# ericyinyzy/VQAttack

Hardware: AMD Instinct MI355X
Metric: adversarial_vqa_examples_per_sec (higher is better)
Workload: dtype f32; 1 GPU; vlmo_base VQAttack image PGD (BASELINE configs[1]): batch 64 per GPU, 40 PGD steps, 384x384 images, questions of 6..14 real tokens ([CLS] + n words + [SEP], n ~ U{4..12} seeded) padded to 40 (the all-padding columns are not run through the encoder), eps 0.125 step 0.01 L-inf clip [-1,1], random start, sanity_checks on, black-box scoring + ASR gather; batch_per_gpu=64, pgd_steps=40, image_size=384, text_len=40, substitutable_words=0

## Files before the change

### include/vqattack_hip.h

```cpp
#ifndef VQATTACK_HIP_H
#define VQATTACK_HIP_H

#include <stddef.h>
#include <stdint.h>

#ifdef __cplusplus
extern "C" {
#endif

typedef void* vqa_stream_t;

#define VQA_OK 0
#define VQA_ERR_NULL (-1)
#define VQA_ERR_SHAPE (-2)
#define VQA_ERR_ALIGN (-3)

#define VQA_CLIP 1u
#define VQA_CHECK_RANGE 2u
#define VQA_FLAG_RANGE 1
#define VQA_FLAG_BAD_LABEL 2
#define VQA_FLAG_DEGENERATE 4

int vqa_abi_version(void);
const char* vqa_error_string(int code);
// ... 54 lines not shown
int vqa_neg_cos_max_layers(void);
int vqa_neg_cos_rows_multi(const float* const* a, const float* const* b, float* const* ga, int n_layers,
                           float* partial, const uint8_t* row_mask, long mask_period, long rows0, long rows1, int D,
                           long a_stride0, long a_stride1, long b_stride0, long b_stride1, long g_stride0,
                           long g_stride1, float gscale, float cos_eps, float* loss_out, int accumulate,
                           vqa_stream_t stream);

int vqa_sum_partials(const float* partial, int count, float* dst, int accumulate, float scale,
                     vqa_stream_t stream);

int vqa_ce_max_label_sets(void);
long vqa_ce_scratch_floats(int K, long groups);
int vqa_ce_rows(const float* logits, long row_stride, const int64_t* labels, int K, long rows, int V,
                long ignore_index, long rows_per_group, float* scratch, float* grad, float* row_loss, float gscale,
                float* loss_out, int accumulate, int* flag, unsigned char* row_state, vqa_stream_t stream);

int vqa_gather_rows(const float* src, const int64_t* idx, float* dst, int B, int L, int K, int D,
                    vqa_stream_t stream);

int vqa_cand_dir_sim(const float* word, const float* pos, const float* type, const float* gamma,
                     const float* beta, float ln_eps, const float* e_ori, const float* grad,
                     const int32_t* cand, float* out, int n_cand, int L, int K, int D, vqa_stream_t stream);

int vqa_embed_tokens(const float* word, const float* pos, const float* type, const float* gamma, const float* beta,
                     float ln_eps, const int32_t* triples, int n, float* dst, int D, vqa_stream_t stream);

int vqa_greedy_accept(const int32_t* cand, const int32_t* order, const int32_t* seg, int B, int L,
                      const int64_t* ori_ids, int64_t* cur_ids, int32_t* new_id, int32_t* acc_rank, const float* table,
                      int V, int E, float threshold, vqa_stream_t stream);

int vqa_attn_fwd(const float* q, const float* k, const float* v, const float* bias, float* o, float* lse, float* scores,
                 int B, int H, int Sq, int Sk, const long* strides, const long* bias_strides, float scale,
                 const int* key_hole, int nsplit, float* split_ws, vqa_stream_t stream);
long vqa_attn_scores_floats(int B, int H, int Sq, int Sk);
long vqa_attn_split_ws_floats(int B, int H, int Sq, int Sk, int nsplit);

int vqa_attn_bwd(const float* q, const float* k, const float* v, const float* bias, const float* o, const float* go,
                 const float* lse, const float* scores, float* delta, float* dq, float* dk, float* dv, float* ds_ws, int B,
                 int H, int Sq, int Sk, const long* strides, const long* bias_strides, const long* grad_strides,
                 float scale, int nsplit, float* split_ws, vqa_stream_t stream);
long vqa_attn_bwd_ws_floats(int B, int H, int Sq, int Sk);

int vqa_resize_bicubic_h_u8(const uint8_t* src, int h, int w_in, int c, const int32_t* kk, const int32_t* bounds,
                            int ksize, int w_out, uint8_t* dst, vqa_stream_t stream);
int vqa_resize_bicubic_v_normalize(const uint8_t* src, int h_in, int w, int c, const int32_t* kk,
                                   const int32_t* bounds, int ksize, int h_out, float mean, float stdv, float* dst,
                                   vqa_stream_t stream);

int vqa_ln_fwd(const float* x, const float* r0, const float* r1, const float* rscale, float* x_out,
               const float* gamma0, const float* beta0, const float* gamma1, const float* beta1, float* y0, float* y1,
               float* mean, float* rstd, long rows, int D, long period, long split, float eps, vqa_stream_t stream);
int vqa_ln_bwd(const float* dy0, const float* dy1, const float* x, const float* mean, const float* rstd,
               const float* gamma0, const float* gamma1, const float* g_a, const float* g_inj, const float* rscale,
               float* dx, float* dr0, float* dr1, long rows, int D, long period, long split, vqa_stream_t stream);
int vqa_ln_bwd_post(const float* dy_a, const float* dy_b, const float* g_inj, const float* s, const float* rstd,
                    const float* gamma, float* ds, long rows, int D, vqa_stream_t stream);
int vqa_gelu_fwd(const float* h, float* a, size_t n, vqa_stream_t stream);
int vqa_gelu_bwd(const float* h, const float* da, float* dh, size_t n, vqa_stream_t stream);

size_t vqa_gemm_packed_bytes(int K, int N);
int vqa_gemm_pack_b(const float* w, long ldw, int trans, void* packed, int K, int N, vqa_stream_t stream);
int vqa_gemm_bf16x6(const float* A, long lda, const void* packed, const float* bias, float* C, long ldc, long M, int N,
                    int K, vqa_stream_t stream);

size_t vqa_gemm_small_ws_bytes(long M, int N, int ksplit);
int vqa_gemm_bf16x6_small(const float* A, long lda, const void* packed, const float* bias, float* C, long ldc, long M,
// ... 7 lines not shown
```

### vqattack_amd/_hip.py

```python
import ctypes
import os
import threading

import torch

_HERE = os.path.dirname(os.path.abspath(__file__))
LIB_PATH = os.path.join(_HERE, "lib", "libvqattack_hip.so")
TUNING_LIB_PATH = os.path.join(_HERE, "lib", "libvqattack_hip_tuning.so")

VQA_CLIP = 1
VQA_CHECK_RANGE = 2
VQA_FLAG_RANGE = 1
VQA_FLAG_BAD_LABEL = 2
VQA_FLAG_DEGENERATE = 4
ABI_VERSION = 4

_c_float_p = ctypes.c_void_p
_sz = ctypes.c_size_t
_f = ctypes.c_float
_i = ctypes.c_int
_u = ctypes.c_uint
_l = ctypes.c_long
_p = ctypes.c_void_p

SIGNATURES = {
    "vqa_abi_version": (_i, []),
    "vqa_error_string": (ctypes.c_char_p, [_i]),
    "vqa_linf_init": (_i, [_p, _p, _p, _sz, _f, _f, _f, _u, _p, _p]),
    "vqa_linf_fgm": (_i, [_p, _p, _p, _sz, _f, _f, _f, _u, _p, _p]),
    "vqa_linf_step": (_i, [_p, _p, _p, _p, _sz, _f, _f, _f, _f, _u, _p, _p]),
    "vqa_linf_project": (_i, [_p, _p, _p, _sz, _f, _f, _f, _u, _p]),
    "vqa_clip_eta_linf": (_i, [_p, _p, _sz, _f, _p]),
    "vqa_optimize_linear_linf": (_i, [_p, _p, _sz, _f, _p]),
    "vqa_zero_out_clipped_grads": (_i, [_p, _p, _p, _sz, _f, _f, _p]),
    "vqa_reduce_ws_bytes": (_sz, [_i, _sz]),
    "vqa_sumsq_per_sample": (_i, [_p, _p, _p, _i, _sz, _p, _p]),
    "vqa_absmax_ties_per_sample": (_i, [_p, _p, _p, _i, _sz, _p, _p]),
    "vqa_l2_fgm": (_i, [_p, _p, _p, _p, _i, _sz, _f, _f, _f, _u, _p, _p]),
    "vqa_l2_project": (_i, [_p, _p, _p, _p, _i, _sz, _f, _f, _f, _u, _p]),
    "vqa_l1_fgm": (_i, [_p, _p, _p, _p, _p, _i, _sz, _f, _f, _f, _u, _p, _p]),
    "vqa_scale_per_sample": (_i, [_p, _p, _p, _p, _i, _sz, _f, _i, _p, _p]),
    "vqa_neg_cos_partials": (_i, []),
    "vqa_neg_cos_rows": (_i, [_p, _p, _p, _p, _p, _l, _l, _l, _i, _l, _l, _l, _l, _l, _l, _f, _f, _p, _i, _p]),
    "vqa_neg_cos_max_layers": (_i, []),
    "vqa_neg_cos_rows_multi": (_i, [_p, _p, _p, _i, _p, _p, _l, _l, _l, _i, _l, _l, _l, _l, _l, _l, _f, _f, _p, _i, _p]),
    "vqa_sum_partials": (_i, [_p, _i, _p, _i, _f, _p]),
    "vqa_ce_max_label_sets": (_i, []),
    "vqa_ce_scratch_floats": (_l, [_i, _l]),
    "vqa_ce_rows": (_i, [_p, _l, _p, _i, _l, _i, _l, _l, _p, _p, _p, _f, _p, _i, _p, _p, _p]),
    "vqa_gather_rows": (_i, [_p, _p, _p, _i, _i, _i, _i, _p]),
    "vqa_cand_dir_sim": (_i, [_p, _p, _p, _p, _p, _f, _p, _p, _p, _p, _i, _i, _i, _i, _p]),
    "vqa_embed_tokens": (_i, [_p, _p, _p, _p, _p, _f, _p, _i, _p, _i, _p]),
    "vqa_greedy_accept": (_i, [_p, _p, _p, _i, _i, _p, _p, _p, _p, _p, _i, _i, _f, _p]),
    "vqa_attn_fwd": (_i, [_p, _p, _p, _p, _p, _p, _p, _i, _i, _i, _i, _p, _p, _f, _p, _i, _p, _p]),
    "vqa_attn_split_ws_floats": (_l, [_i, _i, _i, _i, _i]),
    "vqa_attn_scores_floats": (_l, [_i, _i, _i, _i]),
    "vqa_attn_bwd": (_i, [_p, _p, _p, _p, _p, _p, _p, _p, _p, _p, _p, _p, _p, _i, _i, _i, _i, _p, _p, _p, _f, _i, _p, _p]),
    "vqa_attn_bwd_ws_floats": (_l, [_i, _i, _i, _i]),
    "vqa_ln_fwd": (_i, [_p] * 13 + [_l, _i, _l, _l, _f, _p]),
    "vqa_ln_bwd": (_i, [_p] * 13 + [_l, _i, _l, _l, _p]),
    "vqa_ln_bwd_post": (_i, [_p] * 7 + [_l, _i, _p]),
    "vqa_gelu_fwd": (_i, [_p, _p, _sz, _p]),
    "vqa_gelu_bwd": (_i, [_p, _p, _p, _sz, _p]),
    "vqa_resize_bicubic_h_u8": (_i, [_p, _i, _i, _i, _p, _p, _i, _i, _p, _p]),
    "vqa_resize_bicubic_v_normalize": (_i, [_p, _i, _i, _i, _p, _p, _i, _i, _f, _f, _p, _p]),
    "vqa_gemm_packed_bytes": (_sz, [_i, _i]),
    "vqa_gemm_pack_b": (_i, [_p, _l, _i, _p, _i, _i, _p]),
    "vqa_gemm_bf16x6": (_i, [_p, _l, _p, _p, _p, _l, _l, _i, _i, _p]),
    "vqa_gemm_small_ws_bytes": (_sz, [_l, _i, _i]),
    "vqa_gemm_bf16x6_small": (_i, [_p, _l, _p, _p, _p, _l, _l, _i, _i, _i, _p, _p]),
}

_lib = None
_lock = threading.Lock()


class HipExtensionError(RuntimeError):
    pass


def load_library(path=None):
    tuning = os.environ.get("VQA_TUNING_LIB", "") not in ("", "0")
    if path is None:
        path = TUNING_LIB_PATH if tuning else LIB_PATH
    if not os.path.exists(path):
        raise HipExtensionError(
            "HIP kernel library not found at {} -- build it with `python -m vqattack_amd.build` "
# ... 79 lines not shown
```

### vqattack_amd/attention.py

```python
import ctypes

import torch

from . import _hip
from ._hip import check, lib, ptr, stream_for

HEAD_DIM = 64


def _bshd(t, name):
    if not t.is_cuda or t.dtype != torch.float32 or t.dim() != 4 or t.shape[-1] != HEAD_DIM:
        raise _hip.HipExtensionError("{} must be a float32 (B, S, H, 64) HIP tensor, got {} {}".format(
            name, t.dtype, tuple(t.shape)))
    if t.stride(-1) != 1 or any(s % 4 for s in t.stride()[:-1]) or t.data_ptr() % 16:
        t = t.contiguous()
    return t


def _bias_view(bias, b, h, sq, sk):
    if bias is None:
        return None, None
    if bias.dtype != torch.float32 or not bias.is_cuda:
        raise TypeError("bias must be a float32 HIP tensor")
    bias, in_place = _bias_layout(bias, sk)
# ... 34 lines not shown

    def dense(self):
        sk = self.slab.shape[-1]
        b = self.hole.shape[0]
        keys = torch.arange(sk, device=self.slab.device)
        masked = (keys[None, :] >= self.hole[:, :1]) & (keys[None, :] < self.hole[:, 1:2])
        pad = torch.zeros(b, 1, 1, sk, device=self.slab.device).masked_fill(masked[:, None, None, :], float("-inf"))
        return self.slab + pad


def _split_hole(bias):
    if isinstance(bias, KeyHoleBias):
        return bias.slab, bias.hole
    return bias, None


_CUS = {}


def loop_split(b, h, sq, sk, device, backward=True):
    import os
    pinned = os.environ.get("VQA_ATTN_SPLIT")
    tiles = ((min(sq, sk) if backward else sk) + 31) // 32
    if pinned:
        return max(1, min(int(pinned), tiles))
    dev = torch.device(device).index or 0
    if dev not in _CUS:
        _CUS[dev] = torch.cuda.get_device_properties(dev).multi_processor_count
    wgs = b * h * ((max(sq, sk) + 127) // 128)
    want = 2 * _CUS[dev]
    if wgs * 2 > want:
        return 1
    return max(1, min(8, tiles // 2, -(-want // wgs)))


def _split_ws(b, h, sq, sk, nsplit, device):
    if nsplit <= 1:
        return None
    return torch.empty(int(lib().vqa_attn_split_ws_floats(b, h, sq, sk, nsplit)), dtype=torch.float32, device=device)


def _forward(q, k, v, bias, bstr, scale, save_scores=False, key_hole=None):
    b, sq, h, _ = q.shape
    sk = k.shape[1]
    nsplit = loop_split(b, h, sq, sk, q.device, backward=False)
    sws = _split_ws(b, h, sq, sk, nsplit, q.device)
    o = torch.empty((b, sq, h, HEAD_DIM), dtype=torch.float32, device=q.device)
    lse = torch.empty((b, h, sq), dtype=torch.float32, device=q.device)
    scores = None
    if save_scores:
        if scores_fit(b, h, sq, sk):
            scores = torch.empty(int(lib().vqa_attn_scores_floats(b, h, sq, sk)), dtype=torch.float32, device=q.device)
        elif key_hole is not None:
            raise _hip.HipExtensionError("a key hole needs the saved-scores backward (the recomputing forms read the "
                                         "padding from the bias): pass KeyHoleBias.dense() at this size")
    strides = _longs([q.stride(0), q.stride(1), q.stride(2), k.stride(0), k.stride(1), k.stride(2),
                      v.stride(0), v.stride(1), v.stride(2), o.stride(0), o.stride(1), o.stride(2)])
    if key_hole is not None and (key_hole.dtype != torch.int32 or tuple(key_hole.shape) != (b, 2) or
                                 not key_hole.is_cuda or not key_hole.is_contiguous()):
        raise TypeError("key_hole must be a contiguous int32 (B, 2) HIP tensor")
    with torch.cuda.device(q.device):
        check(lib().vqa_attn_fwd(ptr(q), ptr(k), ptr(v), ptr(bias), ptr(o), ptr(lse), ptr(scores), b, h, sq, sk, strides,
                                 _longs(bstr) if bstr else None, scale,
                                 None if key_hole is None else ctypes.c_void_p(key_hole.data_ptr()), nsplit, ptr(sws),
                                 stream_for(q)),
              "vqa_attn_fwd")
    return o, lse, scores


def scores_fit(b, h, sq, sk):
    n = int(lib().vqa_attn_scores_floats(b, h, sq, sk))
    return 0 < 4 * n <= SCORES_LIMIT and 0 < 4 * int(lib().vqa_attn_bwd_ws_floats(b, h, sq, sk)) <= DS_WORKSPACE_LIMIT


def _prepare(q, k, v, bias, scale, need_grad=False):
    q, k, v = _bshd(q, "q"), _bshd(k, "k"), _bshd(v, "v")
    b, sq, h, _ = q.shape
    sk = k.shape[1]
    if k.shape != (b, sk, h, HEAD_DIM) or v.shape != k.shape:
        raise ValueError("q / k / v shape mismatch: {} {} {}".format(tuple(q.shape), tuple(k.shape), tuple(v.shape)))
    hole = None
    if isinstance(bias, KeyHoleBias):
        if need_grad and not scores_fit(b, h, sq, sk):
            bias = bias.dense()
        else:
            bias, hole = bias.slab, bias.hole
    bias, bstr = _bias_view(bias, b, h, sq, sk)
    return q, k, v, bias, bstr, HEAD_DIM ** -0.5 if scale is None else float(scale), hole


def attention_forward(q, k, v, bias=None, scale=None):
    q, k, v, bias, bstr, scale, hole = _prepare(q, k, v, bias, scale)
    return _forward(q, k, v, bias, bstr, scale, key_hole=hole)[:2]


DS_WORKSPACE_LIMIT = 8 << 30
SCORES_LIMIT = 6 << 30


# ... 80 lines not shown
```

### vqattack_amd/build.py

```python
import os
import shutil
import subprocess
import sys

HERE = os.path.dirname(os.path.abspath(__file__))
SRC_DIR = os.path.join(HERE, "csrc")
LIB_DIR = os.path.join(HERE, "lib")
LIB_PATH = os.path.join(LIB_DIR, "libvqattack_hip.so")
TUNING_LIB_PATH = os.path.join(LIB_DIR, "libvqattack_hip_tuning.so")
SOURCES = ["linf.hip", "lnorm.hip", "loss.hip", "ce.hip", "text.hip", "image.hip", "attn.hip", "block.hip", "gemm.hip"]
FLAGS = ["-O3", "--offload-arch=gfx950", "-ffp-contract=off", "-fPIC", "-shared", "-std=c++17",
         "-Wall", "-Wno-unused-function"]


KERNEL_SOURCES = (("stream4_kernel", "linf.hip"), ("neg_cos_rows", "loss.hip"), ("ce_rows", "ce.hip"), ("ce_count", "ce.hip"),
                  ("attn_", "attn.hip"), ("sumsq", "lnorm.hip"), ("absmax", "lnorm.hip"), ("per_sample", "lnorm.hip"),
                  ("sum_stage2", "lnorm.hip"), ("ln_fwd", "block.hip"), ("ln_bwd", "block.hip"), ("gelu", "block.hip"),
                  ("resize", "image.hip"), ("gather_rows", "text.hip"), ("cand_dir_sim", "text.hip"),
                  ("embed_tokens", "text.hip"), ("greedy_accept", "text.hip"), ("gemm_", "gemm.hip"))


def kernel_source_digest(kernel_name):
    import hashlib
    src = next((f for key, f in KERNEL_SOURCES if key in kernel_name), None)
    if src is None:
        return None
    h = hashlib.sha256(" ".join(FLAGS).encode())
    for path in (os.path.join(SRC_DIR, src), os.path.join(SRC_DIR, "common.hpp"),
                 os.path.join(HERE, "..", "include", "vqattack_hip.h")):
        with open(path, "rb") as fh:
            h.update(fh.read())
    return h.hexdigest()


def _hipcc():
    for cand in (os.environ.get("HIPCC"), shutil.which("hipcc"), "/opt/rocm/bin/hipcc"):
        if cand and os.path.exists(cand):
            return cand
    raise RuntimeError("hipcc not found: the HIP kernels of vqattack_amd cannot be built")


def _stale(path=LIB_PATH):
    if not os.path.exists(path):
        return True
    built = os.path.getmtime(path)
    deps = [os.path.join(SRC_DIR, f) for f in os.listdir(SRC_DIR)]
    deps.append(os.path.join(HERE, "..", "include", "vqattack_hip.h"))
    return any(os.path.getmtime(d) > built for d in deps)


def build(force=False, verbose=False, tuning=False):
    target = TUNING_LIB_PATH if tuning else LIB_PATH
    if not force and not _stale(target):
        return target
    os.makedirs(LIB_DIR, exist_ok=True)
    cmd = [_hipcc()] + FLAGS + (["-DVQA_TUNING"] if tuning else []) + \
        [os.path.join(SRC_DIR, s) for s in SOURCES] + ["-o", target + ".tmp"]
    if verbose:
        print(" ".join(cmd))
    proc = subprocess.run(cmd, capture_output=True, text=True)
    if proc.returncode != 0:
# ... 13 lines not shown
```

### vqattack_amd/csrc/attn.hip

```cpp
#include "common.hpp"

namespace vqa {

typedef float f32x4 __attribute__((ext_vector_type(4)));
typedef float f32x16 __attribute__((ext_vector_type(16)));

constexpr int kTile = 32;
constexpr int kKs = 65;

struct AttnDims {
  int B, H, Sq, Sk;
  long q_sb, q_ss, q_sh;
  long k_sb, k_ss, k_sh;
  long v_sb, v_ss, v_sh;
  long o_sb, o_ss, o_sh;
  long bias_sb, bias_sh, bias_sr;
  float scale;
};

#ifdef VQA_TUNING
__device__ int d_attn_ablate = 0;
#define VQA_ABLATE(bit) (d_attn_ablate & (bit))
__device__ unsigned long long* d_attn_stamps = nullptr;
#define VQA_STAMP_DECL unsigned long long stamp_t = 0, stamp_sum[8] = {0, 0, 0, 0, 0, 0, 0, 0}; const bool stamp_on = d_attn_stamps != nullptr;
#define VQA_STAMP_START()                                                                              \
  do {                                                                                                 \
    if (stamp_on) {                                                                                    \
      __builtin_amdgcn_sched_barrier(0);                                                               \
      asm volatile("s_memtime %0\n\ts_waitcnt lgkmcnt(0)" : "=s"(stamp_t)::"memory");                  \
      __builtin_amdgcn_sched_barrier(0);                                                               \
    }                                                                                                  \
  } while (0)
#define VQA_STAMP(seg)                                                                                 \
// ... 261 lines not shown
        const float m_new = grow ? mx : m;
        const float mc_new = m_new * kLog2e;
        const float alpha = m == -INFINITY ? 0.0f : __builtin_amdgcn_exp2f(mc - mc_new);
        m = m_new;
        mc = grow ? mc_new : mc;
        l *= alpha;
#pragma unroll
        for (int i = 0; i < 16; ++i) {
          o0[i] *= alpha;
          o1[i] *= alpha;
        }
      }
#pragma unroll
      for (int i = 0; i < 16; ++i) {
        st[i] = __builtin_amdgcn_exp2f(__builtin_fmaf(st[i], kLog2e, -mc));
        l += st[i];
      }
      VQA_STAMP(2);
#pragma unroll
      for (int i = 0; i < 16; ++i) {
        const f32x2 vv = *reinterpret_cast<const f32x2*>(Vs + ((i & 3) + 8 * (i >> 2)) * kVi);
        o0 = mfma(vv[0], st[i], o0);
        o1 = mfma(vv[1], st[i], o1);
      }
      VQA_STAMP(3);
      bcur = bnext;
    }
    if (more) {
      store_tile<kKs>(Kbuf[(kt + 1) & 1], tk, 1.0f);
      store_tile_interleaved(Vbuf[(kt + 1) & 1], tv, 1.0f);
    }
    VQA_STAMP(4);
    if (STORE_S && active && !VQA_ABLATE(1)) {
#pragma unroll
      for (int g = 0; g < 4; ++g)
        *reinterpret_cast<f32x4*>(scp + static_cast<long>(kt) * kBlockFloats + 256 * g) =
            f32x4{sraw[4 * g], sraw[4 * g + 1], sraw[4 * g + 2], sraw[4 * g + 3]};
    }
    VQA_STAMP(5);
    __syncthreads();
    VQA_STAMP(6);
  }
  if (active) VQA_STAMP_FLUSH(0, n_tiles - t_lo);
  if (SPLIT) {
    if (qi < d.Sq) {
      l = halves_sum(l);
      const long row = (static_cast<long>(b) * d.H + head) * d.Sq + qi;
      float* wo = sp.ws + (row * nsp + part) * 64;
#pragma unroll
      for (int g = 0; g < 4; ++g) {
        const int dim = 8 * g + 4 * h;
        *reinterpret_cast<f32x4*>(wo + dim) = f32x4{o0[4 * g], o0[4 * g + 1], o0[4 * g + 2], o0[4 * g + 3]};
        *reinterpret_cast<f32x4*>(wo + 32 + dim) = f32x4{o1[4 * g], o1[4 * g + 1], o1[4 * g + 2], o1[4 * g + 3]};
      }
      if (h == 0) {
        float* ml = sp.ws + static_cast<long>(d.B) * d.H * d.Sq * nsp * 64 + (row * nsp + part) * 2;
        ml[0] = m == -INFINITY ? -INFINITY : mc;
        ml[1] = l;
      }
    }
    return;
  }
  if (qi < d.Sq) {
    l = halves_sum(l);
    const float inv = 1.0f / l;
    float* op = o + b * d.o_sb + head * d.o_sh + static_cast<long>(qi) * d.o_ss;
// ... 511 lines not shown
static int check_attn(const float* q, const float* k, const float* v, const AttnDims& d) {
  if (!q || !k || !v) return VQA_ERR_NULL;
  if (d.B < 0 || d.H <= 0 || d.Sq <= 0 || d.Sk <= 0 || d.H > 65535 || d.B > 65535) return VQA_ERR_SHAPE;
  const long blocks = ((d.Sq > d.Sk ? d.Sq : d.Sk) + 127L) / 128;
  if (blocks * d.H * d.B > 2147483647L) return VQA_ERR_SHAPE;
  if ((d.q_sb | d.q_ss | d.q_sh | d.k_sb | d.k_ss | d.k_sh | d.v_sb | d.v_ss | d.v_sh | d.o_sb | d.o_ss | d.o_sh) & 3)
    return VQA_ERR_SHAPE;
  if (!aligned16(q) || !aligned16(k) || !aligned16(v)) return VQA_ERR_ALIGN;
  return VQA_OK;
}

long vqa_attn_scores_floats(int B, int H, int Sq, int Sk) {
  if (B < 0 || H <= 0 || Sq <= 0 || Sk <= 0) return 0;
  return static_cast<long>(B) * H * sc_rows(Sq) * sc_pitch(Sk);
}

long vqa_attn_split_ws_floats(int B, int H, int Sq, int Sk, int nsplit) {
  if (B < 0 || H <= 0 || Sq <= 0 || Sk <= 0 || nsplit < 1) return 0;
  if (nsplit == 1) return 0;
  const long rq = static_cast<long>(B) * H * Sq, rk = static_cast<long>(B) * H * Sk;
  const long fwd = split_fwd_floats(rq, nsplit), dkv = 2 * split_sum_floats(rk, nsplit), dq = split_sum_floats(rq, nsplit);
  return fwd > dkv ? (fwd > dq ? fwd : dq) : (dkv > dq ? dkv : dq);
}

static int check_split(int nsplit, const float* split_ws, int tiles, long wgs) {
  if (nsplit < 1) return VQA_ERR_SHAPE;
  if (nsplit == 1) return VQA_OK;
  if (!split_ws) return VQA_ERR_NULL;
  if (!aligned16(split_ws)) return VQA_ERR_ALIGN;
  if (nsplit > tiles || wgs * nsplit > 2147483647L) return VQA_ERR_SHAPE;
  return VQA_OK;
}

int vqa_attn_fwd(const float* q, const float* k, const float* v, const float* bias, float* o, float* lse, float* scores,
                 int B, int H, int Sq, int Sk, const long* strides, const long* bias_strides, float scale,
                 const int* key_hole, int nsplit, float* split_ws, vqa_stream_t stream) {
  clear_stale_error();
  if (!strides || !o || !lse || (bias && !bias_strides)) return VQA_ERR_NULL;
  AttnDims d{B, H, Sq, Sk, strides[0], strides[1], strides[2], strides[3], strides[4], strides[5], strides[6],
             strides[7], strides[8], strides[9], strides[10], strides[11], 0, 0, 0, scale};
  if (bias) {
    d.bias_sb = bias_strides[0];
    d.bias_sh = bias_strides[1];
    d.bias_sr = bias_strides[2];
    if (((d.bias_sb | d.bias_sh | d.bias_sr) & 3) || !aligned16(bias)) return VQA_ERR_ALIGN;
  }
  int rc = check_attn(q, k, v, d);
  if (rc != VQA_OK) return rc;
  if (!aligned16(o) || !aligned16(scores)) return VQA_ERR_ALIGN;
  const long wgs = ((Sq + 127L) / 128) * H * B;
  rc = check_split(nsplit, split_ws, (Sk + kTile - 1) / kTile, wgs);
  if (rc != VQA_OK) return rc;
  if (B == 0) return VQA_OK;
  const dim3 grid(static_cast<unsigned>(wgs * nsplit));
  hipStream_t st = static_cast<hipStream_t>(stream);
  const SplitArgs sp{nsplit, split_ws};
  if (nsplit > 1) {
    if (bias && scores) attn_fwd_kernel<true, true, true><<<grid, kBlock, 0, st>>>(q, k, v, bias, o, lse, scores, d, key_hole, sp);
    else if (bias) attn_fwd_kernel<true, false, true><<<grid, kBlock, 0, st>>>(q, k, v, bias, o, lse, scores, d, key_hole, sp);
    else if (scores) attn_fwd_kernel<false, true, true><<<grid, kBlock, 0, st>>>(q, k, v, bias, o, lse, scores, d, key_hole, sp);
    else attn_fwd_kernel<false, false, true><<<grid, kBlock, 0, st>>>(q, k, v, bias, o, lse, scores, d, key_hole, sp);
    const long rows = static_cast<long>(B) * H * Sq;
    attn_fwd_combine_kernel<<<dim3(static_cast<unsigned>((rows + kBlock / 16 - 1) / (kBlock / 16))), kBlock, 0, st>>>(
        split_ws, nsplit, o, lse, d);
    return launch_status();
  }
  if (bias && scores) attn_fwd_kernel<true, true><<<grid, kBlock, 0, st>>>(q, k, v, bias, o, lse, scores, d, key_hole, sp);
  else if (bias) attn_fwd_kernel<true, false><<<grid, kBlock, 0, st>>>(q, k, v, bias, o, lse, scores, d, key_hole, sp);
  else if (scores) attn_fwd_kernel<false, true><<<grid, kBlock, 0, st>>>(q, k, v, bias, o, lse, scores, d, key_hole, sp);
  else attn_fwd_kernel<false, false><<<grid, kBlock, 0, st>>>(q, k, v, bias, o, lse, scores, d, key_hole, sp);
  return launch_status();
}

long vqa_attn_bwd_ws_floats(int B, int H, int Sq, int Sk) {
  if (B < 0 || H <= 0 || Sq <= 0 || Sk <= 0) return 0;
  return static_cast<long>(B) * H * ds_rows(Sk) * ds_pitch(Sq);
}

int vqa_attn_bwd(const float* q, const float* k, const float* v, const float* bias, const float* o, const float* go,
                 const float* lse, const float* scores, float* delta, float* dq, float* dk, float* dv, float* ds_ws, int B,
                 int H, int Sq, int Sk, const long* strides, const long* bias_strides, const long* grad_strides,
                 float scale, int nsplit, float* split_ws, vqa_stream_t stream) {
  clear_stale_error();
  if (!strides || !grad_strides || !o || !go || !lse || !delta || !dq || !dk || !dv || (bias && !bias_strides))
    return VQA_ERR_NULL;
  AttnDims d{B, H, Sq, Sk, strides[0], strides[1], strides[2], strides[3], strides[4], strides[5], strides[6],
             strides[7], strides[8], strides[9], strides[10], strides[11], 0, 0, 0, scale};
  if (bias) {
    d.bias_sb = bias_strides[0];
    d.bias_sh = bias_strides[1];
    d.bias_sr = bias_strides[2];
    if (((d.bias_sb | d.bias_sh | d.bias_sr) & 3) || !aligned16(bias)) return VQA_ERR_ALIGN;
    if (d.bias_sr < 0 || (static_cast<long>(Sq) + 4) * d.bias_sr + Sk >= 2147483647L) return VQA_ERR_SHAPE;
  }
  const int rc = check_attn(q, k, v, d);
  if (rc != VQA_OK) return rc;
  long any = 0;
  for (int i = 0; i < 12; ++i) any |= grad_strides[i];
  if (any & 3) return VQA_ERR_SHAPE;
  if (!aligned16(o) || !aligned16(go) || !aligned16(dq) || !aligned16(dk) || !aligned16(dv) || !aligned16(ds_ws) ||
      !aligned16(scores))
    return VQA_ERR_ALIGN;
  if (ds_ws && (ds_rows(Sk) * ds_pitch(Sq) >= 2147483647L || sc_rows(Sq) * sc_pitch(Sk) >= 2147483647L))
    return VQA_ERR_SHAPE;
// ... 73 lines not shown
```

### vqattack_amd/csrc/gemm.hip

```cpp
#include "common.hpp"

namespace vqa {

typedef __bf16 bf16x8 __attribute__((ext_vector_type(8)));
typedef __bf16 bf16x2 __attribute__((ext_vector_type(2)));
typedef float f32x4 __attribute__((ext_vector_type(4)));
typedef float f32x2 __attribute__((ext_vector_type(2)));

constexpr int kGemmBM = 256, kGemmBN = 128, kGemmBK = 32;
constexpr int kGemmThreads = 512;
constexpr int kGemmMT = kGemmBM / 16, kGemmNT = kGemmBN / 16;
constexpr int kTileBytes = 64 * 16;
constexpr int kGemmABytes = kGemmMT * 3 * kTileBytes;
constexpr int kGemmBBytes = kGemmNT * 3 * kTileBytes;
constexpr int kGemmStage = kGemmABytes + kGemmBBytes;
constexpr int kGemmBPieces = kGemmBBytes / 16 / kGemmThreads;

__device__ __forceinline__ void split2(f32x2 a, bf16x2& h0, bf16x2& h1, bf16x2& h2) {
  h0 = __builtin_convertvector(a, bf16x2);
  f32x2 r = a - __builtin_convertvector(h0, f32x2);
  r.x = __builtin_isfinite(r.x) ? r.x : 0.0f;
  r.y = __builtin_isfinite(r.y) ? r.y : 0.0f;
  h1 = __builtin_convertvector(r, bf16x2);
  h2 = __builtin_convertvector(r - __builtin_convertvector(h1, f32x2), bf16x2);
}

__device__ __forceinline__ void split8(const f32x4& lo, const f32x4& hi, bf16x8& p0, bf16x8& p1, bf16x8& p2) {
  bf16x2 a[4], b[4], c[4];
  split2(f32x2{lo.x, lo.y}, a[0], b[0], c[0]);
  split2(f32x2{lo.z, lo.w}, a[1], b[1], c[1]);
  split2(f32x2{hi.x, hi.y}, a[2], b[2], c[2]);
  split2(f32x2{hi.z, hi.w}, a[3], b[3], c[3]);
  p0 = bf16x8{a[0].x, a[0].y, a[1].x, a[1].y, a[2].x, a[2].y, a[3].x, a[3].y};
  p1 = bf16x8{b[0].x, b[0].y, b[1].x, b[1].y, b[2].x, b[2].y, b[3].x, b[3].y};
  p2 = bf16x8{c[0].x, c[0].y, c[1].x, c[1].y, c[2].x, c[2].y, c[3].x, c[3].y};
}

struct GemmArgs {
  const float* A;
  const bf16x8* B;
  const float* bias;
  float* C;
  long lda, ldc, M;
  int N, K;
};

__global__ __launch_bounds__(kGemmThreads) void gemm_bf16x6_kernel(GemmArgs g) {
  __shared__ __attribute__((aligned(16))) char smem[2 * kGemmStage];
  const int tid = threadIdx.x, lane = tid & 63, wave = tid >> 6;
  const int wm = wave >> 1, wn = wave & 1;
  const int ntb = g.N / kGemmBN;
  const int mtb = static_cast<int>((g.M + kGemmBM - 1) / kGemmBM);
  const int nwg = mtb * ntb, orig = blockIdx.x, xcd = orig & 7, q = nwg >> 3, rem = nwg & 7;
  const int wg = (xcd < rem ? xcd * (q + 1) : rem * (q + 1) + (xcd - rem) * q) + (orig >> 3);
  const int mb = wg / ntb, nb = wg - mb * ntb;
  const long m0 = static_cast<long>(mb) * kGemmBM;
  const int n0 = nb * kGemmBN;
  const int nk = g.K / kGemmBK;
  const int nt16 = g.N / 16;

  const float* arow[2];
#pragma unroll
  for (int j = 0; j < 2; ++j) {
    long r = m0 + (2 * wave + j) * 16 + (lane & 15);
    r = r < g.M ? r : g.M - 1;
    arow[j] = g.A + r * g.lda + 8 * (lane >> 4);
  }
  const bf16x8* bsrc = g.B + static_cast<size_t>(nb) * kGemmNT * 3 * 64;
  const size_t bstep = static_cast<size_t>(nt16) * 3 * 64;
// ... 291 lines not shown
```

Before: 14.31 examples/s.

## Add bf16x6 split-precision MFMA attention forward kernel as default for long queries

Adds a forward attention kernel that splits fp32 Q, K, V and the probabilities into three bf16 pieces and accumulates six bf16 MFMA products per tile. K and V tiles are split into LDS once per tile, double-buffered, with the next tile prefetched into registers. The kernel is selected by default when nsplit is 1 and Sq is at least 128, except when the backward pass recomputes scores. The aim is to replace slower fp32 arithmetic with bf16 matrix-core throughput while keeping near-fp32 accuracy, at the cost of extra split work and LDS traffic. Split helpers move to a shared header.

After: 14.44 examples/s, median of 6. About the same (+1.0%).

```diff
diff --git a/include/vqattack_hip.h b/include/vqattack_hip.h
--- a/include/vqattack_hip.h
+++ b/include/vqattack_hip.h
@@ -110,6 +110,9 @@
 int vqa_attn_fwd(const float* q, const float* k, const float* v, const float* bias, float* o, float* lse, float* scores,
                  int B, int H, int Sq, int Sk, const long* strides, const long* bias_strides, float scale,
                  const int* key_hole, int nsplit, float* split_ws, vqa_stream_t stream);
+int vqa_attn_fwd_bf16x6(const float* q, const float* k, const float* v, const float* bias, float* o, float* lse,
+                        float* scores, int B, int H, int Sq, int Sk, const long* strides, const long* bias_strides,
+                        float scale, const int* key_hole, int nsplit, float* split_ws, vqa_stream_t stream);
 long vqa_attn_scores_floats(int B, int H, int Sq, int Sk);
 long vqa_attn_split_ws_floats(int B, int H, int Sq, int Sk, int nsplit);
 
diff --git a/vqattack_amd/_hip.py b/vqattack_amd/_hip.py
--- a/vqattack_amd/_hip.py
+++ b/vqattack_amd/_hip.py
@@ -53,6 +53,7 @@
     "vqa_embed_tokens": (_i, [_p, _p, _p, _p, _p, _f, _p, _i, _p, _i, _p]),
     "vqa_greedy_accept": (_i, [_p, _p, _p, _i, _i, _p, _p, _p, _p, _p, _i, _i, _f, _p]),
     "vqa_attn_fwd": (_i, [_p, _p, _p, _p, _p, _p, _p, _i, _i, _i, _i, _p, _p, _f, _p, _i, _p, _p]),
+    "vqa_attn_fwd_bf16x6": (_i, [_p, _p, _p, _p, _p, _p, _p, _i, _i, _i, _i, _p, _p, _f, _p, _i, _p, _p]),
     "vqa_attn_split_ws_floats": (_l, [_i, _i, _i, _i, _i]),
     "vqa_attn_scores_floats": (_l, [_i, _i, _i, _i]),
     "vqa_attn_bwd": (_i, [_p, _p, _p, _p, _p, _p, _p, _p, _p, _p, _p, _p, _p, _i, _i, _i, _i, _p, _p, _p, _f, _i, _p, _p]),
diff --git a/vqattack_amd/attention.py b/vqattack_amd/attention.py
--- a/vqattack_amd/attention.py
+++ b/vqattack_amd/attention.py
@@ -90,6 +90,19 @@
     if wgs * 2 > want:
         return 1
     return max(1, min(8, tiles // 2, -(-want // wgs)))
+
+
+FWD_BF16X6_DEFAULT = lambda nsplit, sq: nsplit == 1 and sq >= 128
+
+
+def _forward_entry(nsplit, sq, recomputing_backward):
+    import os
+    mode = os.environ.get("VQA_ATTN", "")
+    if mode not in ("", "fp32", "bf16x6"):
+        raise ValueError("VQA_ATTN must be 'fp32' or 'bf16x6', got '{}'".format(mode))
+    if not recomputing_backward and (mode == "bf16x6" or (mode == "" and FWD_BF16X6_DEFAULT(nsplit, sq))):
+        return lib().vqa_attn_fwd_bf16x6, "vqa_attn_fwd_bf16x6"
+    return lib().vqa_attn_fwd, "vqa_attn_fwd"
 
 
 def _split_ws(b, h, sq, sk, nsplit, device):
@@ -117,12 +130,13 @@
     if key_hole is not None and (key_hole.dtype != torch.int32 or tuple(key_hole.shape) != (b, 2) or
                                  not key_hole.is_cuda or not key_hole.is_contiguous()):
         raise TypeError("key_hole must be a contiguous int32 (B, 2) HIP tensor")
+    entry, name = _forward_entry(nsplit, sq, save_scores and scores is None)
     with torch.cuda.device(q.device):
-        check(lib().vqa_attn_fwd(ptr(q), ptr(k), ptr(v), ptr(bias), ptr(o), ptr(lse), ptr(scores), b, h, sq, sk, strides,
-                                 _longs(bstr) if bstr else None, scale,
-                                 None if key_hole is None else ctypes.c_void_p(key_hole.data_ptr()), nsplit, ptr(sws),
-                                 stream_for(q)),
-              "vqa_attn_fwd")
+        check(entry(ptr(q), ptr(k), ptr(v), ptr(bias), ptr(o), ptr(lse), ptr(scores), b, h, sq, sk, strides,
+                    _longs(bstr) if bstr else None, scale,
+                    None if key_hole is None else ctypes.c_void_p(key_hole.data_ptr()), nsplit, ptr(sws),
+                    stream_for(q)),
+              name)
     return o, lse, scores
 
 
diff --git a/vqattack_amd/build.py b/vqattack_amd/build.py
--- a/vqattack_amd/build.py
+++ b/vqattack_amd/build.py
@@ -26,7 +26,7 @@
     if src is None:
         return None
     h = hashlib.sha256(" ".join(FLAGS).encode())
-    for path in (os.path.join(SRC_DIR, src), os.path.join(SRC_DIR, "common.hpp"),
+    for path in (os.path.join(SRC_DIR, src), os.path.join(SRC_DIR, "common.hpp"), os.path.join(SRC_DIR, "split.hpp"),
                  os.path.join(HERE, "..", "include", "vqattack_hip.h")):
         with open(path, "rb") as fh:
             h.update(fh.read())
diff --git a/vqattack_amd/csrc/attn.hip b/vqattack_amd/csrc/attn.hip
--- a/vqattack_amd/csrc/attn.hip
+++ b/vqattack_amd/csrc/attn.hip
@@ -1,4 +1,7 @@
+#include <type_traits>
+
 #include "common.hpp"
+#include "split.hpp"
 
 namespace vqa {
 
@@ -326,6 +329,244 @@
     }
     VQA_STAMP(4);
     if (STORE_S && active && !VQA_ABLATE(1)) {
+#pragma unroll
+      for (int g = 0; g < 4; ++g)
+        *reinterpret_cast<f32x4*>(scp + static_cast<long>(kt) * kBlockFloats + 256 * g) =
+            f32x4{sraw[4 * g], sraw[4 * g + 1], sraw[4 * g + 2], sraw[4 * g + 3]};
+    }
+    VQA_STAMP(5);
+    __syncthreads();
+    VQA_STAMP(6);
+  }
+  if (active) VQA_STAMP_FLUSH(0, n_tiles - t_lo);
+  if (SPLIT) {
+    if (qi < d.Sq) {
+      l = halves_sum(l);
+      const long row = (static_cast<long>(b) * d.H + head) * d.Sq + qi;
+      float* wo = sp.ws + (row * nsp + part) * 64;
+#pragma unroll
+      for (int g = 0; g < 4; ++g) {
+        const int dim = 8 * g + 4 * h;
+        *reinterpret_cast<f32x4*>(wo + dim) = f32x4{o0[4 * g], o0[4 * g + 1], o0[4 * g + 2], o0[4 * g + 3]};
+        *reinterpret_cast<f32x4*>(wo + 32 + dim) = f32x4{o1[4 * g], o1[4 * g + 1], o1[4 * g + 2], o1[4 * g + 3]};
+      }
+      if (h == 0) {
+        float* ml = sp.ws + static_cast<long>(d.B) * d.H * d.Sq * nsp * 64 + (row * nsp + part) * 2;
+        ml[0] = m == -INFINITY ? -INFINITY : mc;
+        ml[1] = l;
+      }
+    }
+    return;
+  }
+  if (qi < d.Sq) {
+    l = halves_sum(l);
+    const float inv = 1.0f / l;
+    float* op = o + b * d.o_sb + head * d.o_sh + static_cast<long>(qi) * d.o_ss;
+#pragma unroll
+    for (int g = 0; g < 4; ++g) {
+      const int dim = 8 * g + 4 * h;
+      f32x4 a = {o0[4 * g] * inv, o0[4 * g + 1] * inv, o0[4 * g + 2] * inv, o0[4 * g + 3] * inv};
+      f32x4 c = {o1[4 * g] * inv, o1[4 * g + 1] * inv, o1[4 * g + 2] * inv, o1[4 * g + 3] * inv};
+      *reinterpret_cast<f32x4*>(op + dim) = a;
+      *reinterpret_cast<f32x4*>(op + 32 + dim) = c;
+    }
+    if (h == 0) lse[(static_cast<long>(b) * d.H + head) * d.Sq + qi] = mc * kLn2 + __logf(l);
+  }
+}
+
+
+constexpr int kXkPlane = 4 * kWave;
+constexpr int kXvPlane = 2 * 2 * kWave;
+constexpr int kPa[6] = {2, 1, 0, 1, 0, 0}, kPb[6] = {0, 1, 2, 0, 1, 0};
+
+__device__ __forceinline__ f32x16 mfma_bf16(bf16x8 a, bf16x8 b, f32x16 c) {
+  return __builtin_amdgcn_mfma_f32_32x32x16_bf16(a, b, c, 0, 0, 0);
+}
+
+struct SplitTileRegs {
+  f32x4 k[2];
+  f32x2 v[4];
+};
+
+template <bool HAS_BIAS, bool STORE_S, bool SPLIT = false>
+__global__ __launch_bounds__(kBlock, 2) void attn_fwd_bf16x6_kernel(const float* __restrict__ q,
+                                                                    const float* __restrict__ k,
+                                                                    const float* __restrict__ v,
+                                                                    const float* __restrict__ bias,
+                                                                    float* __restrict__ o, float* __restrict__ lse,
+                                                                    float* __restrict__ scores, AttnDims d,
+                                                                    const int* __restrict__ key_hole, SplitArgs sp) {
+  __shared__ __attribute__((aligned(16))) bf16x8 Kp[2][3 * kXkPlane];
+  __shared__ __attribute__((aligned(16))) bf16x8 Vp[2][3 * kXvPlane];
+  const int lane = threadIdx.x & (kWave - 1), wave = threadIdx.x / kWave;
+  const int r = lane & 31, h = lane >> 5;
+  const int nsp = SPLIT ? sp.n : 1;
+  const BlockCoord bc = block_coord(((d.Sq + 127) / 128) * nsp, d.B, d.H);
+  const int b = bc.b, head = bc.head;
+  const int blk = SPLIT ? bc.blk / nsp : bc.blk, part = SPLIT ? bc.blk % nsp : 0;
+  const int q0 = blk * 128 + wave * kTile;
+  const bool active = q0 < d.Sq;
+  const int qi = q0 + r;
+  const int ql = qi < d.Sq ? qi : d.Sq - 1;
+  const float* qp = q + b * d.q_sb + head * d.q_sh + static_cast<long>(ql) * d.q_ss + 8 * h;
+  const float* kb = k + b * d.k_sb + head * d.k_sh;
+  const float* vb = v + b * d.v_sb + head * d.v_sh;
+  const float* bp = HAS_BIAS ? bias + b * d.bias_sb + head * d.bias_sh + static_cast<long>(ql) * d.bias_sr + 4 * h
+                             : nullptr;
+  float* scp = STORE_S ? scores + (static_cast<long>(b) * d.H + head) * sc_rows(d.Sq) * sc_pitch(d.Sk) +
+                             (q0 / kTile) * sc_pitch(d.Sk) * kTile + 4 * lane
+                       : nullptr;
+  bf16x8 qa[3][4];
+#pragma unroll
+  for (int s = 0; s < 4; ++s) {
+    const f32x4 lo = *reinterpret_cast<const f32x4*>(qp + 16 * s), hi = *reinterpret_cast<const f32x4*>(qp + 16 * s + 4);
+    split8<kSplitSigned>(lo * d.scale, hi * d.scale, qa[0][s], qa[1][s], qa[2][s]);
+  }
+  f32x16 o0 = {0}, o1 = {0};
+  float m = -INFINITY, mc = 0.0f, l = 0.0f;
+  const int all_tiles = (d.Sk + kTile - 1) / kTile;
+  const int t_lo = SPLIT ? part * all_tiles / nsp : 0;
+  const int n_tiles = SPLIT ? (part + 1) * all_tiles / nsp : all_tiles;
+  const int hole_lo = key_hole ? key_hole[2 * b] : 0, hole_hi = key_hole ? key_hole[2 * b + 1] : 0;
+  f32x16 bcur = {0};
+  if (HAS_BIAS && active) bcur = load_bias_tile(bp, t_lo * kTile);
+
+  const int last_tile = all_tiles - 1;
+  const int krow = threadIdx.x >> 3, kc8 = (threadIdx.x & 7) * 8;
+  const int vpair = threadIdx.x & 31, vgrp = threadIdx.x >> 5;
+  const int krow_last = min(last_tile * kTile + krow, d.Sk - 1) - last_tile * kTile;
+  const unsigned koff = static_cast<unsigned>(krow * static_cast<int>(d.k_ss) + kc8);
+  const unsigned koff_last = static_cast<unsigned>(krow_last * static_cast<int>(d.k_ss) + kc8);
+  unsigned voff[4], voff_last[4];
+#pragma unroll
+  for (int i = 0; i < 4; ++i) {
+    const int row = 4 * vgrp + i, row_last = min(last_tile * kTile + row, d.Sk - 1) - last_tile * kTile;
+    voff[i] = static_cast<unsigned>(row * static_cast<int>(d.v_ss) + 2 * vpair);
+    voff_last[i] = static_cast<unsigned>(row_last * static_cast<int>(d.v_ss) + 2 * vpair);
+  }
+  const long kstep = kTile * d.k_ss, vstep = kTile * d.v_ss;
+  const int kdst = (kc8 >> 4) * kWave + ((kc8 >> 3) & 1) * 32 + krow;
+  const int vdst = (((vgrp >> 2) * 2 + (vpair >> 4)) * kWave + (vgrp & 1) * 32 + ((2 * vpair) & 31)) * 2 + ((vgrp >> 1) & 1);
+  auto load_tile = [&](int tile) {
+    const float* kt_ = kb + tile * kstep;
+    const float* vt_ = vb + tile * vstep;
+    const bool last = tile == last_tile;
+    SplitTileRegs t;
+    const unsigned ko = last ? koff_last : koff;
+    t.k[0] = *reinterpret_cast<const f32x4*>(kt_ + ko);
+    t.k[1] = *reinterpret_cast<const f32x4*>(kt_ + ko + 4);
+#pragma unroll
+    for (int i = 0; i < 4; ++i) t.v[i] = *reinterpret_cast<const f32x2*>(vt_ + (last ? voff_last[i] : voff[i]));
+    return t;
+  };
+  auto split_to_lds = [&](int buf, const SplitTileRegs& t, auto is_signed) {
+    constexpr SplitKind KIND = decltype(is_signed)::value ? kSplitSigned : kSplitFinite;
+    bf16x8 p0, p1, p2;
+    split8<KIND>(t.k[0], t.k[1], p0, p1, p2);
+    bf16x8* kd = Kp[buf] + kdst;
+    kd[0] = p0;
+    kd[kXkPlane] = p1;
+    kd[2 * kXkPlane] = p2;
+    bf16x4* vd = reinterpret_cast<bf16x4*>(Vp[buf]) + vdst;
+#pragma unroll
+    for (int e = 0; e < 2; ++e) {
+      bf16x2 a[2], bb[2], c[2];
+      split2_as<KIND>(f32x2{t.v[0][e], t.v[1][e]}, a[0], bb[0], c[0]);
+      split2_as<KIND>(f32x2{t.v[2][e], t.v[3][e]}, a[1], bb[1], c[1]);
+      vd[2 * e] = bf16x4{a[0].x, a[0].y, a[1].x, a[1].y};
+      vd[2 * e + 2 * kXvPlane] = bf16x4{bb[0].x, bb[0].y, bb[1].x, bb[1].y};
+      vd[2 * e + 4 * kXvPlane] = bf16x4{c[0].x, c[0].y, c[1].x, c[1].y};
+    }
+  };
+  auto store_split = [&](int buf, const SplitTileRegs& t) {
+    int odd = 0;
+#pragma unroll
+    for (int j = 0; j < 2; ++j)
+      odd |= int(bf16_not_finite(f32x2{t.k[j].x, t.k[j].y})) | int(bf16_not_finite(f32x2{t.k[j].z, t.k[j].w})) |
+             int(bf16_not_finite(f32x2{t.v[0][j], t.v[1][j]})) | int(bf16_not_finite(f32x2{t.v[2][j], t.v[3][j]}));
+    if (__builtin_amdgcn_ballot_w64(odd != 0) != 0) split_to_lds(buf, t, std::true_type{});
+    else split_to_lds(buf, t, std::false_type{});
+  };
+  store_split(t_lo & 1, load_tile(t_lo));
+  __syncthreads();
+  VQA_STAMP_DECL
+  VQA_STAMP_START();
+  for (int kt = t_lo; kt < n_tiles; ++kt) {
+    const int k0 = kt * kTile;
+    const bf16x8* Ks = Kp[kt & 1] + lane;
+    const bf16x8* Vs = Vp[kt & 1] + lane;
+    const bool more = kt + 1 < n_tiles;
+    SplitTileRegs tn;
+    if (more) tn = load_tile(kt + 1);
+    f32x16 sraw;
+    if (active) {
+      f32x16 bnext = {0};
+      if (HAS_BIAS && more) bnext = load_bias_tile(bp, k0 + kTile);
+      __builtin_amdgcn_sched_barrier(0);
+      VQA_STAMP(0);
+      f32x16 st = {0};
+#pragma unroll
+      for (int s = 0; s < 4; ++s)
+#pragma unroll
+        for (int t = 0; t < 6; ++t) st = mfma_bf16(Ks[kPa[t] * kXkPlane + kWave * s], qa[kPb[t]][s], st);
+      VQA_STAMP(1);
+      if (HAS_BIAS) st += bcur;
+      if (k0 < hole_hi && k0 + kTile > hole_lo) {
+#pragma unroll
+        for (int i = 0; i < 16; ++i) {
+          const int key = k0 + acc_row(i, h);
+          st[i] = (key >= hole_lo && key < hole_hi) ? -INFINITY : st[i];
+        }
+      }
+      if (STORE_S) sraw = st;
+      if (k0 + kTile > d.Sk) {
+#pragma unroll
+        for (int i = 0; i < 16; ++i) st[i] = k0 + acc_row(i, h) < d.Sk ? st[i] : -INFINITY;
+      }
+      float mx = st[0];
+#pragma unroll
+      for (int i = 1; i < 16; ++i) mx = fmaxf(mx, st[i]);
+      mx = halves_max(mx);
+      const bool grow = mx > m + kLazyMax;
+      if (__builtin_amdgcn_ballot_w64(grow) != 0) {
+        const float m_new = grow ? mx : m;
+        const float mc_new = m_new * kLog2e;
+        const float alpha = m == -INFINITY ? 0.0f : __builtin_amdgcn_exp2f(mc - mc_new);
+        m = m_new;
+        mc = grow ? mc_new : mc;
+        l *= alpha;
+#pragma unroll
+        for (int i = 0; i < 16; ++i) {
+          o0[i] *= alpha;
+          o1[i] *= alpha;
+        }
+      }
+#pragma unroll
+      for (int i = 0; i < 16; ++i) {
+        st[i] = __builtin_amdgcn_exp2f(__builtin_fmaf(st[i], kLog2e, -mc));
+        l += st[i];
+      }
+      VQA_STAMP(2);
+#pragma unroll
+      for (int s = 0; s < 2; ++s) {
+        bf16x2 a[4], bb[4], c[4];
+#pragma unroll
+        for (int j = 0; j < 4; ++j) split2_finite(f32x2{st[8 * s + 2 * j], st[8 * s + 2 * j + 1]}, a[j], bb[j], c[j]);
+        const bf16x8 pf[3] = {bf16x8{a[0].x, a[0].y, a[1].x, a[1].y, a[2].x, a[2].y, a[3].x, a[3].y},
+                              bf16x8{bb[0].x, bb[0].y, bb[1].x, bb[1].y, bb[2].x, bb[2].y, bb[3].x, bb[3].y},
+                              bf16x8{c[0].x, c[0].y, c[1].x, c[1].y, c[2].x, c[2].y, c[3].x, c[3].y}};
+#pragma unroll
+        for (int t = 0; t < 6; ++t) {
+          o0 = mfma_bf16(Vs[kPa[t] * kXvPlane + kWave * (2 * s)], pf[kPb[t]], o0);
+          o1 = mfma_bf16(Vs[kPa[t] * kXvPlane + kWave * (2 * s + 1)], pf[kPb[t]], o1);
+        }
+      }
+      VQA_STAMP(3);
+      bcur = bnext;
+    }
+    if (more) store_split((kt + 1) & 1, tn);
+    VQA_STAMP(4);
+    if (STORE_S && active) {
 #pragma unroll
       for (int g = 0; g < 4; ++g)
         *reinterpret_cast<f32x4*>(scp + static_cast<long>(kt) * kBlockFloats + 256 * g) =
@@ -903,9 +1144,10 @@
   return VQA_OK;
 }
 
-int vqa_attn_fwd(const float* q, const float* k, const float* v, const float* bias, float* o, float* lse, float* scores,
-                 int B, int H, int Sq, int Sk, const long* strides, const long* bias_strides, float scale,
-                 const int* key_hole, int nsplit, float* split_ws, vqa_stream_t stream) {
+static int attn_fwd_launch(bool bf16x6, const float* q, const float* k, const float* v, const float* bias, float* o,
+                           float* lse, float* scores, int B, int H, int Sq, int Sk, const long* strides,
+                           const long* bias_strides, float scale, const int* key_hole, int nsplit, float* split_ws,
+                           vqa_stream_t stream) {
   clear_stale_error();
   if (!strides || !o || !lse || (bias && !bias_strides)) return VQA_ERR_NULL;
   AttnDims d{B, H, Sq, Sk, strides[0], strides[1], strides[2], strides[3], strides[4], strides[5], strides[6],
@@ -926,21 +1168,40 @@
   const dim3 grid(static_cast<unsigned>(wgs * nsplit));
   hipStream_t st = static_cast<hipStream_t>(stream);
   const SplitArgs sp{nsplit, split_ws};
+  if (bf16x6 && (d.k_ss < 0 || d.v_ss < 0 || d.k_ss >= (1L << 24) || d.v_ss >= (1L << 24))) return VQA_ERR_SHAPE;
+#define VQA_FWD(KERNEL, SPLIT)                                                                                        \
+  do {                                                                                                                \
+    if (bias && scores) KERNEL<true, true, SPLIT><<<grid, kBlock, 0, st>>>(q, k, v, bias, o, lse, scores, d, key_hole, sp);   \
+    else if (bias) KERNEL<true, false, SPLIT><<<grid, kBlock, 0, st>>>(q, k, v, bias, o, lse, scores, d, key_hole, sp);       \
+    else if (scores) KERNEL<false, true, SPLIT><<<grid, kBlock, 0, st>>>(q, k, v, bias, o, lse, scores, d, key_hole, sp);     \
+    else KERNEL<false, false, SPLIT><<<grid, kBlock, 0, st>>>(q, k, v, bias, o, lse, scores, d, key_hole, sp);                \
+  } while (0)
   if (nsplit > 1) {
-    if (bias && scores) attn_fwd_kernel<true, true, true><<<grid, kBlock, 0, st>>>(q, k, v, bias, o, lse, scores, d, key_hole, sp);
-    else if (bias) attn_fwd_kernel<true, false, true><<<grid, kBlock, 0, st>>>(q, k, v, bias, o, lse, scores, d, key_hole, sp);
-    else if (scores) attn_fwd_kernel<false, true, true><<<grid, kBlock, 0, st>>>(q, k, v, bias, o, lse, scores, d, key_hole, sp);
-    else attn_fwd_kernel<false, false, true><<<grid, kBlock, 0, st>>>(q, k, v, bias, o, lse, scores, d, key_hole, sp);
+    if (bf16x6) VQA_FWD(attn_fwd_bf16x6_kernel, true);
+    else VQA_FWD(attn_fwd_kernel, true);
     const long rows = static_cast<long>(B) * H * Sq;
     attn_fwd_combine_kernel<<<dim3(static_cast<unsigned>((rows + kBlock / 16 - 1) / (kBlock / 16))), kBlock, 0, st>>>(
         split_ws, nsplit, o, lse, d);
     return launch_status();
   }
-  if (bias && scores) attn_fwd_kernel<true, true><<<grid, kBlock, 0, st>>>(q, k, v, bias, o, lse, scores, d, key_hole, sp);
-  else if (bias) attn_fwd_kernel<true, false><<<grid, kBlock, 0, st>>>(q, k, v, bias, o, lse, scores, d, key_hole, sp);
-  else if (scores) attn_fwd_kernel<false, true><<<grid, kBlock, 0, st>>>(q, k, v, bias, o, lse, scores, d, key_hole, sp);
-  else attn_fwd_kernel<false, false><<<grid, kBlock, 0, st>>>(q, k, v, bias, o, lse, scores, d, key_hole, sp);
+  if (bf16x6) VQA_FWD(attn_fwd_bf16x6_kernel, false);
+  else VQA_FWD(attn_fwd_kernel, false);
+#undef VQA_FWD
   return launch_status();
+}
+
+int vqa_attn_fwd(const float* q, const float* k, const float* v, const float* bias, float* o, float* lse, float* scores,
+                 int B, int H, int Sq, int Sk, const long* strides, const long* bias_strides, float scale,
+                 const int* key_hole, int nsplit, float* split_ws, vqa_stream_t stream) {
+  return attn_fwd_launch(false, q, k, v, bias, o, lse, scores, B, H, Sq, Sk, strides, bias_strides, scale, key_hole,
+                         nsplit, split_ws, stream);
+}
+
+int vqa_attn_fwd_bf16x6(const float* q, const float* k, const float* v, const float* bias, float* o, float* lse,
+                        float* scores, int B, int H, int Sq, int Sk, const long* strides, const long* bias_strides,
+                        float scale, const int* key_hole, int nsplit, float* split_ws, vqa_stream_t stream) {
+  return attn_fwd_launch(true, q, k, v, bias, o, lse, scores, B, H, Sq, Sk, strides, bias_strides, scale, key_hole,
+                         nsplit, split_ws, stream);
 }
 
 long vqa_attn_bwd_ws_floats(int B, int H, int Sq, int Sk) {
diff --git a/vqattack_amd/csrc/gemm.hip b/vqattack_amd/csrc/gemm.hip
--- a/vqattack_amd/csrc/gemm.hip
+++ b/vqattack_amd/csrc/gemm.hip
@@ -1,9 +1,8 @@
 #include "common.hpp"
+#include "split.hpp"
 
 namespace vqa {
 
-typedef __bf16 bf16x8 __attribute__((ext_vector_type(8)));
-typedef __bf16 bf16x2 __attribute__((ext_vector_type(2)));
 typedef float f32x4 __attribute__((ext_vector_type(4)));
 typedef float f32x2 __attribute__((ext_vector_type(2)));
 
@@ -15,26 +14,6 @@
 constexpr int kGemmBBytes = kGemmNT * 3 * kTileBytes;
 constexpr int kGemmStage = kGemmABytes + kGemmBBytes;
 constexpr int kGemmBPieces = kGemmBBytes / 16 / kGemmThreads;
-
-__device__ __forceinline__ void split2(f32x2 a, bf16x2& h0, bf16x2& h1, bf16x2& h2) {
-  h0 = __builtin_convertvector(a, bf16x2);
-  f32x2 r = a - __builtin_convertvector(h0, f32x2);
-  r.x = __builtin_isfinite(r.x) ? r.x : 0.0f;
-  r.y = __builtin_isfinite(r.y) ? r.y : 0.0f;
-  h1 = __builtin_convertvector(r, bf16x2);
-  h2 = __builtin_convertvector(r - __builtin_convertvector(h1, f32x2), bf16x2);
-}
-
-__device__ __forceinline__ void split8(const f32x4& lo, const f32x4& hi, bf16x8& p0, bf16x8& p1, bf16x8& p2) {
-  bf16x2 a[4], b[4], c[4];
-  split2(f32x2{lo.x, lo.y}, a[0], b[0], c[0]);
-  split2(f32x2{lo.z, lo.w}, a[1], b[1], c[1]);
-  split2(f32x2{hi.x, hi.y}, a[2], b[2], c[2]);
-  split2(f32x2{hi.z, hi.w}, a[3], b[3], c[3]);
-  p0 = bf16x8{a[0].x, a[0].y, a[1].x, a[1].y, a[2].x, a[2].y, a[3].x, a[3].y};
-  p1 = bf16x8{b[0].x, b[0].y, b[1].x, b[1].y, b[2].x, b[2].y, b[3].x, b[3].y};
-  p2 = bf16x8{c[0].x, c[0].y, c[1].x, c[1].y, c[2].x, c[2].y, c[3].x, c[3].y};
-}
 
 struct GemmArgs {
   const float* A;
diff --git a/vqattack_amd/csrc/split.hpp b/vqattack_amd/csrc/split.hpp
--- /dev/null
+++ b/vqattack_amd/csrc/split.hpp
@@ -0,0 +1,70 @@
+#pragma once
+#include "common.hpp"
+
+namespace vqa {
+
+typedef __bf16 bf16x8 __attribute__((ext_vector_type(8)));
+typedef __bf16 bf16x4 __attribute__((ext_vector_type(4)));
+typedef __bf16 bf16x2 __attribute__((ext_vector_type(2)));
+typedef float f32x4 __attribute__((ext_vector_type(4)));
+typedef float f32x2 __attribute__((ext_vector_type(2)));
+
+__device__ __forceinline__ void split2(f32x2 a, bf16x2& h0, bf16x2& h1, bf16x2& h2) {
+  h0 = __builtin_convertvector(a, bf16x2);
+  f32x2 r = a - __builtin_convertvector(h0, f32x2);
+  r.x = __builtin_isfinite(r.x) ? r.x : 0.0f;
+  r.y = __builtin_isfinite(r.y) ? r.y : 0.0f;
+  h1 = __builtin_convertvector(r, bf16x2);
+  h2 = __builtin_convertvector(r - __builtin_convertvector(h1, f32x2), bf16x2);
+}
+
+__device__ __forceinline__ bool bf16_not_finite(f32x2 a) {
+  const f32x2 a0 = __builtin_convertvector(__builtin_convertvector(a, bf16x2), f32x2);
+  return !__builtin_isfinite(a0.x) || !__builtin_isfinite(a0.y);
+}
+
+__device__ __forceinline__ void split2_signed(f32x2 a, bf16x2& h0, bf16x2& h1, bf16x2& h2) {
+  f32x2 a0 = __builtin_convertvector(__builtin_convertvector(a, bf16x2), f32x2);
+  const bool nx = !__builtin_isfinite(a0.x), ny = !__builtin_isfinite(a0.y);
+  f32x2 r = a - a0;
+  r.x = nx ? 0.0f : r.x;
+  r.y = ny ? 0.0f : r.y;
+  h1 = __builtin_convertvector(r, bf16x2);
+  f32x2 r2 = r - __builtin_convertvector(h1, f32x2);
+  r2.x = nx ? a0.x : r2.x;
+  r2.y = ny ? a0.y : r2.y;
+  h2 = __builtin_convertvector(r2, bf16x2);
+  a0.x = nx ? 0.0f : a0.x;
+  a0.y = ny ? 0.0f : a0.y;
+  h0 = __builtin_convertvector(a0, bf16x2);
+}
+
+__device__ __forceinline__ void split2_finite(f32x2 a, bf16x2& h0, bf16x2& h1, bf16x2& h2) {
+  h0 = __builtin_convertvector(a, bf16x2);
+  const f32x2 r = a - __builtin_convertvector(h0, f32x2);
+  h1 = __builtin_convertvector(r, bf16x2);
+  h2 = __builtin_convertvector(r - __builtin_convertvector(h1, f32x2), bf16x2);
+}
+
+enum SplitKind { kSplitGuarded, kSplitSigned, kSplitFinite };
+
+template <SplitKind KIND = kSplitGuarded>
+__device__ __forceinline__ void split2_as(f32x2 a, bf16x2& h0, bf16x2& h1, bf16x2& h2) {
+  if (KIND == kSplitSigned) split2_signed(a, h0, h1, h2);
+  else if (KIND == kSplitFinite) split2_finite(a, h0, h1, h2);
+  else split2(a, h0, h1, h2);
+}
+
+template <SplitKind KIND = kSplitGuarded>
+__device__ __forceinline__ void split8(const f32x4& lo, const f32x4& hi, bf16x8& p0, bf16x8& p1, bf16x8& p2) {
+  bf16x2 a[4], b[4], c[4];
+  split2_as<KIND>(f32x2{lo.x, lo.y}, a[0], b[0], c[0]);
+  split2_as<KIND>(f32x2{lo.z, lo.w}, a[1], b[1], c[1]);
+  split2_as<KIND>(f32x2{hi.x, hi.y}, a[2], b[2], c[2]);
+  split2_as<KIND>(f32x2{hi.z, hi.w}, a[3], b[3], c[3]);
+  p0 = bf16x8{a[0].x, a[0].y, a[1].x, a[1].y, a[2].x, a[2].y, a[3].x, a[3].y};
+  p1 = bf16x8{b[0].x, b[0].y, b[1].x, b[1].y, b[2].x, b[2].y, b[3].x, b[3].y};
+  p2 = bf16x8{c[0].x, c[0].y, c[1].x, c[1].y, c[2].x, c[2].y, c[3].x, c[3].y};
+}
+
+}
```
